# bioinfomaticsCSU/deepsignal

Measured on AMD Instinct MI355X. Metric: CpG sites/sec (batch=512, k=17, sig=360), higher is better.
Workload: dtype f32; 1 GPU; configs[1]: 1xMI355X, batch=512, random-init CpG model weights, synthetic (17,360) features, fp32; batch=512, kmer_len=17, signal_len=360

## Files before the change

deepsignal_amd/csrc/ds_kernels.hip:

```cpp
#include "ds_device.h"

namespace ds {


constexpr int DR_SLOTS = 4;
constexpr int DR_DIST = 3;
constexpr int DR_STAGE = 6 * 256;
constexpr int DR_A_FLOATS = 2 * 128 * (KC + 4);
constexpr int DR_LDS_FLOATS = DR_A_FLOATS + DR_SLOTS * DR_STAGE + 2 * 256;
constexpr int DR_SOLO_PAD_BYTES = 56 * 1024;

__device__ __forceinline__ void dr_gload4(v4f& dst, unsigned voff, const void* sbase)
{
    asm volatile("global_load_dwordx4 %0, %1, %2" : "=&v"(dst) : "v"(voff), "s"(sbase) : "memory");
}
template <int E> __device__ __forceinline__ float dr_elem(const v4f& v) { return E == 0 ? v.x : E == 1 ? v.y : E == 2 ? v.z : v.w; }

__device__ __forceinline__ void dense_ring_loop(const GemmProblem& P, float* smem, int m0, int tid, int lane, int wave,
                                                int t0, int t1, int t2, floatx16 (&acc)[1][3])
{
    constexpr int LDA = KC + 4;
    const int nchunks = P.K / KC;
    if (nchunks <= 0) return;
    float* const ring = smem + DR_A_FLOATS;
// ... 1788 lines not shown
    const int W = a.W, spt = a.spt;
    const int trows = spt * (W + 2) + 3;
    int* const rowmap = reinterpret_cast<int*>(T + trows * S23_LDT);
    const int site0 = blockIdx.x * spt;
    const int nhere = min(spt, a.n_sites - site0);
    const int TRv = nhere * W;
    const size_t grow0 = (size_t)site0 * W;
    const int h4 = 4 * (lane >> 5), rlane = lane & 31;

    for (int i = tid; i < trows * (S23_LDT / 4); i += 512) reinterpret_cast<float4*>(T)[i] = make_float4(0.f, 0.f, 0.f, 0.f);
    if (tid < 96) rowmap[tid] = tid < TRv ? (tid / W) * (W + 2) + 1 + tid % W : spt * (W + 2) + 1;
    {
        float4 v[3];
#pragma unroll
        for (int i = 0; i < 3; ++i) {
            const int idx = tid + 512 * i, row = idx >> 4, q = idx & 15;
            const int rr = row < TRv ? row : TRv - 1;
            v[i] = gload4(a.X + (grow0 + rr) * 64 + q * 4);
        }
#pragma unroll
        for (int i = 0; i < 3; ++i) {
            const int idx = tid + 512 * i, row = idx >> 4, q = idx & 15;
            *reinterpret_cast<float4*>(Xs + row * S23_LDX + q * 4) = v[i];
        }
    }
    const char* const b3 = reinterpret_cast<const char*>(a.Bp3) + (size_t)wave * 48 * 1024;
    const unsigned lane16 = (unsigned)lane * 16;
    float4 bq[4];
#pragma unroll
    for (int i = 0; i < 4; ++i) bq[i] = gload4(reinterpret_cast<const float*>(b3 + i * 1024 + lane16));
    float4 bias3[4];
#pragma unroll
    for (int g = 0; g < 4; ++g) bias3[g] = gload4(a.bias3 + wave * 32 + 8 * g + h4);
    __syncthreads();

    {
        const int n2 = wave & 3;
        float4 w2[8];
#pragma unroll
        for (int g = 0; g < 8; ++g) w2[g] = gload4(a.Bp2 + ((size_t)(n2 * 8 + g) * 64 + lane) * 4);
        float4 bias2[4];
#pragma unroll
        for (int g = 0; g < 4; ++g) bias2[g] = gload4(a.bias2 + n2 * 32 + 8 * g + h4);
        const int nunits = wave < 4 ? 2 : 1;
        for (int ui = 0; ui < nunits; ++ui) {
            const int m = wave < 4 ? 2 * ui : 1;
            floatx16 u;
#pragma unroll
            for (int g = 0; g < 4; ++g) { u[4 * g] = bias2[g].x; u[4 * g + 1] = bias2[g].y; u[4 * g + 2] = bias2[g].z; u[4 * g + 3] = bias2[g].w; }
            const float* xr = Xs + (m * 32 + rlane) * S23_LDX + h4;
#pragma unroll
            for (int g = 0; g < 8; ++g) {
                const float4 x = *reinterpret_cast<const float4*>(xr + g * 8);
                u = __builtin_amdgcn_mfma_f32_32x32x2f32(w2[g].x, x.x, u, 0, 0, 0);
                u = __builtin_amdgcn_mfma_f32_32x32x2f32(w2[g].y, x.y, u, 0, 0, 0);
                u = __builtin_amdgcn_mfma_f32_32x32x2f32(w2[g].z, x.z, u, 0, 0, 0);
                u = __builtin_amdgcn_mfma_f32_32x32x2f32(w2[g].w, x.w, u, 0, 0, 0);
            }
            const int row = m * 32 + rlane;
            float* const td = T + rowmap[row] * S23_LDT + n2 * 32 + h4;
#pragma unroll
            for (int g = 0; g < 4; ++g) {
                const float4 o = make_float4(relu_f(u[4 * g]), relu_f(u[4 * g + 1]), relu_f(u[4 * g + 2]), relu_f(u[4 * g + 3]));
                *reinterpret_cast<float4*>(td + 8 * g) = o;
                if (a.C2 && row < TRv) {
                    const v4f ov = {o.x, o.y, o.z, o.w};
                    *(__attribute__((address_space(1))) v4f*)(a.C2 + (grow0 + row) * 128 + n2 * 32 + 8 * g + h4) = ov;
                }
            }
        }
    }
    __syncthreads();

    floatx16 acc[3];
#pragma unroll
    for (int m = 0; m < 3; ++m)
#pragma unroll
        for (int g = 0; g < 4; ++g) { acc[m][4 * g] = bias3[g].x; acc[m][4 * g + 1] = bias3[g].y; acc[m][4 * g + 2] = bias3[g].z; acc[m][4 * g + 3] = bias3[g].w; }
    const float* tb[3];
#pragma unroll
    for (int m = 0; m < 3; ++m) tb[m] = T + (rowmap[m * 32 + rlane] - 1) * S23_LDT + h4;
    float4 af[2][3];
#pragma unroll
    for (int m = 0; m < 3; ++m) af[0][m] = *reinterpret_cast<const float4*>(tb[m]);
#pragma unroll
    for (int kgl = 0; kgl < 48; ++kgl) {
        const int cur = kgl & 1, slot = kgl & 3;
        if (kgl + 1 < 48) {
            const int t1 = (kgl + 1) >> 4, g1 = (kgl + 1) & 15;
#pragma unroll
            for (int m = 0; m < 3; ++m) af[cur ^ 1][m] = *reinterpret_cast<const float4*>(tb[m] + t1 * S23_LDT + g1 * 8);
        }
#pragma unroll
        for (int m = 0; m < 3; ++m) {
            acc[m] = __builtin_amdgcn_mfma_f32_32x32x2f32(bq[slot].x, af[cur][m].x, acc[m], 0, 0, 0);
            acc[m] = __builtin_amdgcn_mfma_f32_32x32x2f32(bq[slot].y, af[cur][m].y, acc[m], 0, 0, 0);
            acc[m] = __builtin_amdgcn_mfma_f32_32x32x2f32(bq[slot].z, af[cur][m].z, acc[m], 0, 0, 0);
            acc[m] = __builtin_amdgcn_mfma_f32_32x32x2f32(bq[slot].w, af[cur][m].w, acc[m], 0, 0, 0);
        }
        if (kgl + 4 < 48) bq[slot] = gload4(reinterpret_cast<const float*>(b3 + (kgl + 4) * 1024 + lane16));
        __builtin_amdgcn_sched_barrier(0);
    }

#pragma unroll
    for (int m = 0; m < 3; ++m) {
        const int row = m * 32 + rlane;
        if (row < TRv) {
            float* const yd = a.Y + (grow0 + row) * 256 + wave * 32 + h4;
#pragma unroll
            for (int g = 0; g < 4; ++g) {
                const v4f o = {relu_f(acc[m][4 * g]), relu_f(acc[m][4 * g + 1]), relu_f(acc[m][4 * g + 2]), relu_f(acc[m][4 * g + 3])};
                *(__attribute__((address_space(1))) v4f*)(yd + 8 * g) = o;
            }
        }
    }
}

hipError_t launch_stem23(const Stem23Args& a, hipStream_t s)
{
    if (a.n_sites <= 0) return hipSuccess;
    const int grid = (a.n_sites + a.spt - 1) / a.spt;
    hipLaunchKernelGGL(stem23_kernel, dim3(grid), dim3(512), stem23_lds_bytes(a.W, a.spt), s, a);
    return hipGetLastError();
}

constexpr int SB_LDX = 36;
constexpr int SB_LDT = 68;
constexpr int SB_LDO = 132;
size_t stem23_bf16_lds_bytes(int W, int spt)
{
    const size_t work = (size_t)96 * SB_LDX + (size_t)(spt * (W + 2) + 3) * SB_LDT;
    const size_t outt = (size_t)96 * SB_LDO;
    return ((work > outt ? work : outt) + 96) * sizeof(float);
}

__global__ __launch_bounds__(512, 4) void stem23_bf16_kernel(const Stem23Args a)
{
    extern __shared__ __attribute__((aligned(16))) float smem[];
    float* const Xs = smem;
    float* const T = smem + 96 * SB_LDX;
    float* const Ot = smem;
    const int tid = threadIdx.x, lane = tid & 63, wave = __builtin_amdgcn_readfirstlane(tid >> 6);
    const int W = a.W, spt = a.spt;
    const int trows = spt * (W + 2) + 3;
    const size_t work = (size_t)96 * SB_LDX + (size_t)trows * SB_LDT, outt = (size_t)96 * SB_LDO;
    int* const rowmap = reinterpret_cast<int*>(smem + (work > outt ? work : outt));
    const int site0 = blockIdx.x * spt;
    const int TRv = min(spt, a.n_sites - site0) * W;
    const size_t grow0 = (size_t)site0 * W;
    const int h4 = 4 * (lane >> 5), rlane = lane & 31;
    unsigned short* const Th = reinterpret_cast<unsigned short*>(T);
    unsigned short* const Oh = reinterpret_cast<unsigned short*>(Ot);
    auto pack4 = [](float x0, float x1, float x2, float x3) -> uint2 {
        return make_uint2(pack_bf2(relu_f(x0), relu_f(x1)), pack_bf2(relu_f(x2), relu_f(x3)));
    };

    for (int i = tid; i < trows * (SB_LDT / 4); i += 512) reinterpret_cast<float4*>(T)[i] = make_float4(0.f, 0.f, 0.f, 0.f);
    if (tid < 96) rowmap[tid] = tid < TRv ? (tid / W) * (W + 2) + 1 + tid % W : spt * (W + 2) + 1;
    {
        float4 v[2];
#pragma unroll
        for (int i = 0; i < 2; ++i) {
            const int idx = tid + 512 * i, row = idx >> 3, q = idx & 7;
            const int rr = row < TRv ? row : TRv - 1;
            if (idx < 768) v[i] = gload4(a.X + (grow0 + rr) * 32 + q * 4);
        }
#pragma unroll
        for (int i = 0; i < 2; ++i) {
            const int idx = tid + 512 * i, row = idx >> 3, q = idx & 7;
            if (idx < 768) *reinterpret_cast<float4*>(Xs + row * SB_LDX + q * 4) = v[i];
        }
    }
    const char* const b3 = reinterpret_cast<const char*>(a.Bp3) + (size_t)wave * 24 * 1024;
    const unsigned lane16 = (unsigned)lane * 16;
    float4 bq[4];
#pragma unroll
    for (int i = 0; i < 4; ++i) bq[i] = gload4(reinterpret_cast<const float*>(b3 + i * 1024 + lane16));
    float4 bias3[4];
#pragma unroll
    for (int g = 0; g < 4; ++g) bias3[g] = gload4(a.bias3 + wave * 32 + 8 * g + h4);
    __syncthreads();

    {
        const int n2 = wave & 3;
        float4 w2[4];
#pragma unroll
        for (int g = 0; g < 4; ++g) w2[g] = gload4(a.Bp2 + ((size_t)(n2 * 4 + g) * 64 + lane) * 4);
        float4 bias2[4];
#pragma unroll
        for (int g = 0; g < 4; ++g) bias2[g] = gload4(a.bias2 + n2 * 32 + 8 * g + h4);
        const int nunits = wave < 4 ? 2 : 1;
        for (int ui = 0; ui < nunits; ++ui) {
            const int m = wave < 4 ? 2 * ui : 1;
            floatx16 u;
#pragma unroll
            for (int g = 0; g < 4; ++g) { u[4 * g] = bias2[g].x; u[4 * g + 1] = bias2[g].y; u[4 * g + 2] = bias2[g].z; u[4 * g + 3] = bias2[g].w; }
            const float* xr = Xs + (m * 32 + rlane) * SB_LDX + h4;
#pragma unroll
            for (int g = 0; g < 4; ++g) u = mfma_bf(w2[g], *reinterpret_cast<const float4*>(xr + g * 8), u);
            const int row = m * 32 + rlane;
            unsigned short* const td = Th + rowmap[row] * (2 * SB_LDT) + n2 * 32 + h4;
#pragma unroll
            for (int g = 0; g < 4; ++g) {
                const uint2 o = pack4(u[4 * g], u[4 * g + 1], u[4 * g + 2], u[4 * g + 3]);
                *reinterpret_cast<uint2*>(td + 8 * g) = o;
                if (a.C2 && row < TRv) {
                    typedef unsigned int u2v __attribute__((ext_vector_type(2)));
                    const u2v ov = {o.x, o.y};
                    *(__attribute__((address_space(1))) u2v*)(reinterpret_cast<unsigned short*>(a.C2) + (grow0 + row) * 128 + n2 * 32 + 8 * g + h4) = ov;
                }
            }
        }
    }
    __syncthreads();

    floatx16 acc[3];
#pragma unroll
    for (int m = 0; m < 3; ++m)
#pragma unroll
        for (int g = 0; g < 4; ++g) { acc[m][4 * g] = bias3[g].x; acc[m][4 * g + 1] = bias3[g].y; acc[m][4 * g + 2] = bias3[g].z; acc[m][4 * g + 3] = bias3[g].w; }
    const float* tb[3];
#pragma unroll
    for (int m = 0; m < 3; ++m) tb[m] = T + (rowmap[m * 32 + rlane] - 1) * SB_LDT + h4;
    float4 af[3];
#pragma unroll
    for (int m = 0; m < 3; ++m) af[m] = *reinterpret_cast<const float4*>(tb[m]);
#pragma unroll
    for (int ks = 0; ks < 24; ++ks) {
        const int slot = ks & 3;
#pragma unroll
        for (int m = 0; m < 3; ++m) acc[m] = mfma_bf(bq[slot], af[m], acc[m]);
        if (ks + 4 < 24) bq[slot] = gload4(reinterpret_cast<const float*>(b3 + (ks + 4) * 1024 + lane16));
        if (ks + 1 < 24) {
            const int t1 = (ks + 1) >> 3, g1 = (ks + 1) & 7;
#pragma unroll
            for (int m = 0; m < 3; ++m) af[m] = *reinterpret_cast<const float4*>(tb[m] + t1 * SB_LDT + g1 * 8);
        }
        __builtin_amdgcn_sched_barrier(0);
    }
    __syncthreads();

#pragma unroll
    for (int m = 0; m < 3; ++m)
#pragma unroll
        for (int g = 0; g < 4; ++g)
            *reinterpret_cast<uint2*>(Oh + (m * 32 + rlane) * (2 * SB_LDO) + wave * 32 + 8 * g + h4) =
                pack4(acc[m][4 * g], acc[m][4 * g + 1], acc[m][4 * g + 2], acc[m][4 * g + 3]);
    __syncthreads();
    __attribute__((address_space(1))) unsigned short* const Yg =
        (__attribute__((address_space(1))) unsigned short*)(reinterpret_cast<unsigned short*>(a.Y) + grow0 * 256);
    for (int idx = tid; idx < 96 * 32; idx += 512) {
        const int row = idx >> 5, q = idx & 31;
        if (row < TRv) {
            const float4 v = *reinterpret_cast<const float4*>(Ot + row * SB_LDO + q * 4);
            v4f o = {v.x, v.y, v.z, v.w};
            *(__attribute__((address_space(1))) v4f*)(Yg + (unsigned)(row * 256 + q * 8)) = o;
        }
    }
}

hipError_t launch_stem23_bf16(const Stem23Args& a, hipStream_t s)
{
    if (a.n_sites <= 0) return hipSuccess;
    const int grid = (a.n_sites + a.spt - 1) / a.spt;
    hipLaunchKernelGGL(stem23_bf16_kernel, dim3(grid), dim3(512), stem23_bf16_lds_bytes(a.W, a.spt), s, a);
    return hipGetLastError();
}

hipError_t configure_fused_kernels()
{
    const void* fns[6] = {(const void*)inception_fused_kernel<1>, (const void*)inception_fused_kernel<2>,
                          (const void*)inception_fused_kernel<3>, (const void*)inception_fused_bf16_kernel<1>,
                          (const void*)inception_fused_bf16_kernel<2>, (const void*)inception_fused_bf16_kernel<3>};
    for (const void* f : fns) {
        const hipError_t e = hipFuncSetAttribute(f, hipFuncAttributeMaxDynamicSharedMemorySize, 160 * 1024);
        if (e != hipSuccess) return e;
    }
    const hipError_t e1 = hipFuncSetAttribute((const void*)gemm_kernel<1, 3, 4, 1, 0, 2, 2, 1>, hipFuncAttributeMaxDynamicSharedMemorySize, DR_SOLO_PAD_BYTES);
    if (e1 != hipSuccess) return e1;
    const hipError_t e2 = hipFuncSetAttribute((const void*)stem23_bf16_kernel, hipFuncAttributeMaxDynamicSharedMemorySize, (int)STEM23_MAX_LDS);
    if (e2 != hipSuccess) return e2;
    return hipFuncSetAttribute((const void*)stem23_kernel, hipFuncAttributeMaxDynamicSharedMemorySize, (int)STEM23_MAX_LDS);
}

hipError_t launch_inception_fused_bf16(int tm, const FusedChain& c, hipStream_t s)
{
    if (!fused_chain_ok(c)) return hipErrorInvalidValue;
    const FusedArgs& a = c.m[0];
    if (a.n_sites <= 0) return hipSuccess;
    for (int i = 1; i < c.nmod; ++i)
        if (c.m[i].cin != a.cin) return hipErrorInvalidValue;
    const size_t lds = inception_fused_bf16_lds_bytes(tm, a.W, a.spt);
    const int grid = (a.n_sites + a.spt - 1) / a.spt;
    switch (tm) {
    case 1: hipLaunchKernelGGL(inception_fused_bf16_kernel<1>, dim3(grid), dim3(512), lds, s, c); break;
    case 2: hipLaunchKernelGGL(inception_fused_bf16_kernel<2>, dim3(grid), dim3(512), lds, s, c); break;
    case 3: hipLaunchKernelGGL(inception_fused_bf16_kernel<3>, dim3(grid), dim3(512), lds, s, c); break;
    default: return hipErrorInvalidValue;
    }
    return hipGetLastError();
}

constexpr int STEM_HALO = 8;
template <bool OUT_BF>
__global__ __launch_bounds__(256) void stem1_kernel(const float* __restrict__ signals, const float* __restrict__ w,
                                                     const float* __restrict__ bias, float* __restrict__ out,
                                                     int signal_len, int w1, int pad_l_conv, int wa, int pad_l_pool)
{
    extern __shared__ __attribute__((aligned(16))) float sig[];
    const int site = blockIdx.x;
    const int total = signal_len + 2 * STEM_HALO + 8;
    for (int i = threadIdx.x; i < total; i += blockDim.x) {
        const int k = i - STEM_HALO;
        sig[i] = (k >= 0 && k < signal_len) ? signals[(size_t)site * signal_len + k] : 0.0f;
    }
    __syncthreads();
    const int c = threadIdx.x & 63;
    float wk[7];
#pragma unroll
    for (int t = 0; t < 7; ++t) wk[t] = w[t * 64 + c];
    const float b = bias[c];
    for (int p = threadIdx.x >> 6; p < wa; p += blockDim.x >> 6) {
        const int wc0 = 2 * p - pad_l_pool;
        const float* s0 = sig + STEM_HALO + 2 * wc0 - pad_l_conv;
        float v[11];
#pragma unroll
        for (int i = 0; i < 11; ++i) v[i] = s0[i];
        float best = -INFINITY;
#pragma unroll
        for (int pt = 0; pt < 3; ++pt) {
            float a = 0.0f;
#pragma unroll
            for (int t = 0; t < 7; ++t) a = fmaf(v[2 * pt + t], wk[t], a);
            const int wc = wc0 + pt;
            best = (wc >= 0 && wc < w1) ? __builtin_elementwise_maximum(best, a) : best;
        }
        const float y = relu_f(best + b);
        if (OUT_BF) reinterpret_cast<unsigned short*>(out)[((size_t)site * wa + p) * 64 + c] = f2bf(y);
        else out[((size_t)site * wa + p) * 64 + c] = y;
    }
}

hipError_t launch_stem1(const float* signals, const float* w7x64, const float* bias64, float* out, int n,
                        int signal_len, int w1, int pad_l_conv, int wa, int pad_l_pool, int out_bf16, hipStream_t s)
{
    if (n <= 0) return hipSuccess;
    const size_t lds = (signal_len + 2 * STEM_HALO + 8) * sizeof(float);
    if (lds > 64 * 1024) return hipErrorInvalidValue;
    if (out_bf16)
        hipLaunchKernelGGL(stem1_kernel<true>, dim3(n), dim3(256), lds, s, signals, w7x64, bias64, out,
                           signal_len, w1, pad_l_conv, wa, pad_l_pool);
    else
        hipLaunchKernelGGL(stem1_kernel<false>, dim3(n), dim3(256), lds, s, signals, w7x64, bias64, out,
                           signal_len, w1, pad_l_conv, wa, pad_l_pool);
    return hipGetLastError();
}

__global__ __launch_bounds__(256) void maxpool_s2_kernel(const float4* __restrict__ in, float4* __restrict__ out,
                                                          long total, int win, int wout, int pad_l, int ch4)
{
    for (long i = blockIdx.x * (long)blockDim.x + threadIdx.x; i < total; i += (long)gridDim.x * blockDim.x) {
        const int c = (int)(i % ch4);
        const long r = i / ch4;
        const int wo = (int)(r % wout);
        const long site = r / wout;
        float4 m = make_float4(0.0f, 0.0f, 0.0f, 0.0f);
#pragma unroll
        for (int t = 0; t < 3; ++t) {
            const int wi = 2 * wo + t - pad_l;
            if (wi >= 0 && wi < win) m = f4max_relu(m, in[(site * win + wi) * ch4 + c]);
        }
        out[i] = m;
    }
}

hipError_t launch_maxpool_s2(const float* in, float* out, int n, int win, int wout, int pad_l, int ch, hipStream_t s)
{
    const long total = (long)n * wout * (ch / 4);
    if (total <= 0) return hipSuccess;
    const int blocks = (int)((total + 255) / 256 < 4096 ? (total + 255) / 256 : 4096);
    hipLaunchKernelGGL(maxpool_s2_kernel, dim3(blocks), dim3(256), 0, s, (const float4*)in, (float4*)out, total, win, wout,
                       pad_l, ch / 4);
    return hipGetLastError();
}

__global__ __launch_bounds__(256) void avgpool7_kernel(const float4* __restrict__ in, float4* __restrict__ out, long total,
                                                        int w, int ch4)
{
    for (long i = blockIdx.x * (long)blockDim.x + threadIdx.x; i < total; i += (long)gridDim.x * blockDim.x) {
        const int c = (int)(i % ch4);
        const long r = i / ch4;
        const int wo = (int)(r % w);
        const long site = r / w;
        float4 a = make_float4(0.f, 0.f, 0.f, 0.f);
        int cnt = 0;
        for (int t = -3; t <= 3; ++t) {
            const int wi = wo + t;
            if (wi < 0 || wi >= w) continue;
            const float4 v = in[(site * w + wi) * ch4 + c];
            a.x += v.x; a.y += v.y; a.z += v.z; a.w += v.w;
            ++cnt;
        }
        const float d = (float)cnt;
        out[i] = make_float4(a.x / d, a.y / d, a.z / d, a.w / d);
    }
}

hipError_t launch_avgpool7(const float* in, float* out, int n, int w, int ch, hipStream_t s)
{
    const long total = (long)n * w * (ch / 4);
    if (total <= 0) return hipSuccess;
    const int blocks = (int)((total + 255) / 256 < 4096 ? (total + 255) / 256 : 4096);
    hipLaunchKernelGGL(avgpool7_kernel, dim3(blocks), dim3(256), 0, s, (const float4*)in, (float4*)out, total, w, ch / 4);
    return hipGetLastError();
}

__global__ __launch_bounds__(256) void head_kernel(const float* __restrict__ fc1, const float* __restrict__ w2,
                                                    float* __restrict__ logits, float* __restrict__ act,
                                                    int* __restrict__ pred, int n, int J, int C, int nparts, size_t part_stride)
{
    __shared__ float part[4][16];
    const int site = blockIdx.x;
    const int tid = threadIdx.x, lane = tid & 63, wave = tid >> 6;
    const float4* x4 = reinterpret_cast<const float4*>(fc1 + (size_t)site * J);
    float accv[16];
#pragma unroll
    for (int c = 0; c < 16; ++c) accv[c] = 0.0f;
    const int J4 = J >> 2;
    for (int k4 = tid; k4 < J4; k4 += 256) {
        float4 x = x4[k4];
        for (int p = 1; p < nparts; ++p) {
            const float4 y = *reinterpret_cast<const float4*>(fc1 + p * part_stride + (size_t)site * J + 4 * (size_t)k4);
            x.x += y.x; x.y += y.y; x.z += y.z; x.w += y.w;
        }
        const float* w = w2 + (size_t)k4 * 4 * C;
        if (C == 2) {
            const float4 wa = *reinterpret_cast<const float4*>(w);
            const float4 wb = *reinterpret_cast<const float4*>(w + 4);
            accv[0] = fmaf(x.x, wa.x, fmaf(x.y, wa.z, fmaf(x.z, wb.x, fmaf(x.w, wb.z, accv[0]))));
            accv[1] = fmaf(x.x, wa.y, fmaf(x.y, wa.w, fmaf(x.z, wb.y, fmaf(x.w, wb.w, accv[1]))));
        } else {
#pragma unroll
            for (int c = 0; c < 16; ++c)
                if (c < C) accv[c] += x.x * w[c] + x.y * w[C + c] + x.z * w[2 * C + c] + x.w * w[3 * C + c];
        }
    }
    for (int k = (J4 << 2) + tid; k < J; k += 256) {
        float xk = fc1[(size_t)site * J + k];
        for (int p = 1; p < nparts; ++p) xk += fc1[p * part_stride + (size_t)site * J + k];
        for (int c = 0; c < C; ++c) accv[c] += xk * w2[(size_t)k * C + c];
    }
#pragma unroll
    for (int c = 0; c < 16; ++c) {
        if (c >= C) break;
        float a = accv[c];
#pragma unroll
        for (int off = 32; off > 0; off >>= 1) a += __shfl_xor(a, off);
        if (lane == 0) part[wave][c] = a;
    }
    __syncthreads();
    if (tid == 0) {
        float best = 0.0f;
        int bi = 0;
        for (int c = 0; c < C; ++c) {
            const float a = (part[0][c] + part[1][c]) + (part[2][c] + part[3][c]);
            const float sg = sigmoidf_(a);
            logits[(size_t)site * C + c] = a;
            act[(size_t)site * C + c] = sg;
            if (c == 0 || sg > best) { best = sg; bi = c; }
        }
        pred[site] = bi;
    }
}

hipError_t launch_head(const float* fc1, const float* w2, float* logits, float* act, int* pred, int n, int J,
                       int class_num, hipStream_t s, int nparts, size_t part_stride)
{
    if (n <= 0) return hipSuccess;
    hipLaunchKernelGGL(head_kernel, dim3(n), dim3(256), 0, s, fc1, w2, logits, act, pred, n, J, class_num, nparts, part_stride);
    return hipGetLastError();
}

__global__ __launch_bounds__(256) void head_folded_kernel(const HeadFoldedArgs a)
{
    __shared__ float part[4][16];
    const int site = blockIdx.x, C = a.C;
    const int tid = threadIdx.x, lane = tid & 63, wave = tid >> 6;
    float accv[16];
#pragma unroll
    for (int c = 0; c < 16; ++c) accv[c] = 0.0f;
    int koff = 0;
    if (a.bf16) {
        for (int sg = 0; sg < a.nseg; ++sg) {
        const float4* x8 = reinterpret_cast<const float4*>(reinterpret_cast<const unsigned short*>(a.seg[sg]) + (size_t)site * a.pitch[sg]);
        for (int k8 = tid; k8 < (a.len[sg] >> 3); k8 += 256) {
            const float4 raw = x8[k8];
            const unsigned u[4] = {__float_as_uint(raw.x), __float_as_uint(raw.y), __float_as_uint(raw.z), __float_as_uint(raw.w)};
            const float* w = a.w + (size_t)(koff + k8 * 8) * C;
            if (C == 2) {
#pragma unroll
                for (int e = 0; e < 4; ++e) {
                    const float x0 = __uint_as_float(u[e] << 16), x1 = __uint_as_float(u[e] & 0xffff0000u);
                    const float4 wv = *reinterpret_cast<const float4*>(w + 4 * e);
                    accv[0] = fmaf(x0, wv.x, fmaf(x1, wv.z, accv[0]));
                    accv[1] = fmaf(x0, wv.y, fmaf(x1, wv.w, accv[1]));
                }
            } else {
#pragma unroll
                for (int e = 0; e < 4; ++e) {
                    const float x0 = __uint_as_float(u[e] << 16), x1 = __uint_as_float(u[e] & 0xffff0000u);
#pragma unroll
                    for (int c = 0; c < 16; ++c)
                        if (c < C) accv[c] += x0 * w[(2 * e) * C + c] + x1 * w[(2 * e + 1) * C + c];
                }
            }
        }
        koff += a.len[sg];
        }
    } else
    for (int sg = 0; sg < a.nseg; ++sg) {
        const int len = a.len[sg];
        const float4* x4 = reinterpret_cast<const float4*>(a.seg[sg] + (size_t)site * len);
        for (int k4 = tid; k4 < (len >> 2); k4 += 256) {
            const float4 x = x4[k4];
            const float* w = a.w + (size_t)(koff + k4 * 4) * C;
            if (C == 2) {
                const float4 wa = *reinterpret_cast<const float4*>(w);
                const float4 wb = *reinterpret_cast<const float4*>(w + 4);
                accv[0] = fmaf(x.x, wa.x, fmaf(x.y, wa.z, fmaf(x.z, wb.x, fmaf(x.w, wb.z, accv[0]))));
                accv[1] = fmaf(x.x, wa.y, fmaf(x.y, wa.w, fmaf(x.z, wb.y, fmaf(x.w, wb.w, accv[1]))));
            } else {
#pragma unroll
                for (int c = 0; c < 16; ++c)
                    if (c < C) accv[c] += x.x * w[c] + x.y * w[C + c] + x.z * w[2 * C + c] + x.w * w[3 * C + c];
            }
        }
        koff += len;
    }
#pragma unroll
    for (int c = 0; c < 16; ++c) {
        if (c >= C) break;
        float v = accv[c];
#pragma unroll
        for (int off = 32; off > 0; off >>= 1) v += __shfl_xor(v, off);
        if (lane == 0) part[wave][c] = v;
    }
    __syncthreads();
    if (tid == 0) {
        float best = 0.0f;
        int bi = 0;
        for (int c = 0; c < C; ++c) {
            const float v = (part[0][c] + part[1][c]) + (part[2][c] + part[3][c]);
            const float sgm = sigmoidf_(v);
            a.logits[(size_t)site * C + c] = v;
            a.act[(size_t)site * C + c] = sgm;
            if (c == 0 || sgm > best) { best = sgm; bi = c; }
        }
        a.pred[site] = bi;
    }
}

hipError_t launch_head_folded(const HeadFoldedArgs& a, hipStream_t s)
{
    if (a.n <= 0) return hipSuccess;
    hipLaunchKernelGGL(head_folded_kernel, dim3(a.n), dim3(256), 0, s, a);
    return hipGetLastError();
}

__global__ __launch_bounds__(256) void gather_inputs_kernel(const int* __restrict__ kmer, const float* __restrict__ means,
                                                            const float* __restrict__ stds, const float* __restrict__ lens,
                                                            const float* __restrict__ signals, float* __restrict__ block,
                                                            int n, int T, int S, int B, long lo, long hi)
{
    const long nt = (long)n * T;
    const long bt = (long)B * T;
    for (long i = lo + (long)blockIdx.x * 256 + threadIdx.x; i < hi; i += (long)gridDim.x * 256) {
        if (i < nt) reinterpret_cast<int*>(block)[i] = kmer[i];
        else if (i < 2 * nt) block[bt + (i - nt)] = means[i - nt];
        else if (i < 3 * nt) block[2 * bt + (i - 2 * nt)] = stds[i - 2 * nt];
        else if (i < 4 * nt) block[3 * bt + (i - 3 * nt)] = lens[i - 3 * nt];
        else block[4 * bt + (i - 4 * nt)] = signals[i - 4 * nt];
    }
}

__global__ __launch_bounds__(256) void scatter_outputs_kernel(const float* __restrict__ act, const int* __restrict__ pred,
                                                              float* __restrict__ act_out, int* __restrict__ pred_out, int n, int C)
{
    const int total = n * C + n;
    for (int i = blockIdx.x * 256 + threadIdx.x; i < total; i += gridDim.x * 256) {
        if (i < n * C) act_out[i] = act[i];
        else pred_out[i - n * C] = pred[i - n * C];
    }
}

hipError_t launch_gather_inputs(const int* kmer, const float* means, const float* stds, const float* lens, const float* signals,
                                float* block, int n, int T, int S, int B, int col_lo, int col_hi, hipStream_t s)
{
    if (n <= 0 || col_lo < 0 || col_hi > 4 * T + S || col_lo >= col_hi) return hipSuccess;
    const long lo = (long)n * col_lo, hi = (long)n * col_hi;
    const int grid = (int)std::min<long>((hi - lo + 1023) / 1024, 1024);
    hipLaunchKernelGGL(gather_inputs_kernel, dim3(grid), dim3(256), 0, s, kmer, means, stds, lens, signals, block, n, T, S, B, lo, hi);
    return hipGetLastError();
}

hipError_t launch_scatter_outputs(const float* act, const int* pred, float* act_out, int* pred_out, int n, int C, hipStream_t s)
{
    if (n <= 0) return hipSuccess;
    hipLaunchKernelGGL(scatter_outputs_kernel, dim3((n * (C + 1) + 255) / 256), dim3(256), 0, s, act, pred, act_out, pred_out, n, C);
    return hipGetLastError();
}

__global__ __launch_bounds__(256) void maxpool_s2_bf16_kernel(const float4* __restrict__ in, float4* __restrict__ out,
                                                               long total, int win, int wout, int pad_l, int ch8)
{
    for (long i = blockIdx.x * (long)blockDim.x + threadIdx.x; i < total; i += (long)gridDim.x * blockDim.x) {
        const int c = (int)(i % ch8);
        const long r = i / ch8;
        const int wo = (int)(r % wout);
        const long site = r / wout;
        float4 m = make_float4(0.0f, 0.0f, 0.0f, 0.0f);
#pragma unroll
        for (int t = 0; t < 3; ++t) {
            const int wi = 2 * wo + t - pad_l;
            if (wi >= 0 && wi < win) m = bf8max_relu(m, in[(site * win + wi) * ch8 + c]);
        }
        out[i] = m;
    }
}

hipError_t launch_maxpool_s2_bf16(const float* in, float* out, int n, int win, int wout, int pad_l, int ch_ld, hipStream_t s)
{
    const long total = (long)n * wout * (ch_ld / 8);
    if (total <= 0) return hipSuccess;
    const int blocks = (int)((total + 255) / 256 < 8192 ? (total + 255) / 256 : 8192);
    hipLaunchKernelGGL(maxpool_s2_bf16_kernel, dim3(blocks), dim3(256), 0, s, (const float4*)in, (float4*)out, total, win,
                       wout, pad_l, ch_ld / 8);
    return hipGetLastError();
}

__global__ __launch_bounds__(256) void avgpool7_bf16_kernel(const float4* __restrict__ in, unsigned short* __restrict__ out,
                                                             long total, int w, int ch8, int ld_in8, long out_ld, int out_off)
{
    for (long i = blockIdx.x * (long)blockDim.x + threadIdx.x; i < total; i += (long)gridDim.x * blockDim.x) {
        const int c = (int)(i % ch8);
        const long r = i / ch8;
        const int wo = (int)(r % w);
        const long site = r / w;
        float a[8] = {0, 0, 0, 0, 0, 0, 0, 0};
        int cnt = 0;
        for (int t = -3; t <= 3; ++t) {
            const int wi = wo + t;
            if (wi < 0 || wi >= w) continue;
            const float4 v = in[(site * w + wi) * ld_in8 + c];
            const unsigned u[4] = {__float_as_uint(v.x), __float_as_uint(v.y), __float_as_uint(v.z), __float_as_uint(v.w)};
#pragma unroll
            for (int q = 0; q < 4; ++q) {
                a[2 * q] += __uint_as_float(u[q] << 16);
                a[2 * q + 1] += __uint_as_float(u[q] & 0xffff0000u);
            }
            ++cnt;
        }
        const float d = (float)cnt;
        unsigned o[4];
#pragma unroll
        for (int q = 0; q < 4; ++q) o[q] = pack_bf2(a[2 * q] / d, a[2 * q + 1] / d);
        *reinterpret_cast<uint4*>(out + site * out_ld + out_off + ((long)wo * ch8 + c) * 8) = make_uint4(o[0], o[1], o[2], o[3]);
    }
}

hipError_t launch_avgpool7_bf16(const float* in, float* joint, int n, int w, int ch, int ld_in, int joint_ld, int joint_off,
                                hipStream_t s)
{
    const long total = (long)n * w * (ch / 8);
    if (total <= 0) return hipSuccess;
    const int blocks = (int)((total + 255) / 256 < 8192 ? (total + 255) / 256 : 8192);
    hipLaunchKernelGGL(avgpool7_bf16_kernel, dim3(blocks), dim3(256), 0, s, (const float4*)in, (unsigned short*)joint, total, w,
                       ch / 8, ld_in / 8, (long)joint_ld, joint_off);
    return hipGetLastError();
}

template <bool SRC_BF>
__global__ __launch_bounds__(256) void pack_event_feat_bf16_kernel(const float* __restrict__ hfw, const float* __restrict__ hbw,
                                                                    unsigned short* __restrict__ joint, int n, long joint_ld)
{
    const long i = blockIdx.x * (long)blockDim.x + threadIdx.x;
    if (i >= (long)n * 128) return;
    const int site = (int)(i / 128), q = (int)(i % 128);
    uint2 o;
    if (SRC_BF) {
        const unsigned short* src = reinterpret_cast<const unsigned short*>(q < 64 ? hfw : hbw) + (size_t)site * 256 + (q & 63) * 4;
        o = *reinterpret_cast<const uint2*>(src);
    } else {
        const float* src = (q < 64 ? hfw : hbw) + (size_t)site * 256 + (q & 63) * 4;
        const float4 v = *reinterpret_cast<const float4*>(src);
        o = make_uint2(pack_bf2(v.x, v.y), pack_bf2(v.z, v.w));
    }
    *reinterpret_cast<uint2*>(joint + site * joint_ld + q * 4) = o;
}

hipError_t launch_pack_event_feat_bf16(const float* hfw, const float* hbw, float* joint, int n, int joint_ld, int src_bf16,
                                       hipStream_t s)
{
    if (n <= 0) return hipSuccess;
    const dim3 grid((unsigned)(((long)n * 128 + 255) / 256));
    if (src_bf16)
        hipLaunchKernelGGL(pack_event_feat_bf16_kernel<true>, grid, dim3(256), 0, s, hfw, hbw, (unsigned short*)joint, n, (long)joint_ld);
    else
        hipLaunchKernelGGL(pack_event_feat_bf16_kernel<false>, grid, dim3(256), 0, s, hfw, hbw, (unsigned short*)joint, n, (long)joint_ld);
    return hipGetLastError();
}

__global__ __launch_bounds__(256) void embed_table_kernel(const float* __restrict__ emb, const float* __restrict__ kernel,
                                                           float* __restrict__ table, int vocab, int esize, int ncol)
{
    const long i = blockIdx.x * (long)blockDim.x + threadIdx.x;
    if (i >= (long)vocab * ncol) return;
    const int col = (int)(i % ncol);
    const int v = (int)(i / ncol);
    float a = 0.0f;
    for (int e = 0; e < esize; ++e) a = fmaf(emb[(size_t)v * esize + e], kernel[(size_t)e * ncol + col], a);
    table[i] = a;
}

hipError_t launch_embed_table(const float* emb, const float* kernel, float* table, int vocab, int esize, int ncol,
                              hipStream_t s)
{
    const long total = (long)vocab * ncol;
    hipLaunchKernelGGL(embed_table_kernel, dim3((unsigned)((total + 255) / 256)), dim3(256), 0, s, emb, kernel, table, vocab,
                       esize, ncol);
    return hipGetLastError();
}

}
```

Measured before the change: 461,300 sites/s.

## Restructure small kernels: stem1 carry reuse, per-site avgpool, segment-wise gather copies, wave priority

Rewrites several small auxiliary kernels. stem1 now gives each wave a contiguous range of pool outputs and reuses the overlapping conv result and sliding signal window. avgpool7 runs one block per site without per-element div/mod. Gather and scatter become per-segment vectorized uint4 copies. Several kernels raise wave priority with s_setprio and use 32-bit byte offsets for addressing. The aim is to cut index arithmetic and instruction overhead in these minor stages, at the cost of added complexity and new overflow and alignment assumptions.

Measured after the change: 466,800 sites/s, median of 6. +1.2%, better.

```diff
diff --git a/deepsignal_amd/csrc/ds_kernels.hip b/deepsignal_amd/csrc/ds_kernels.hip
--- a/deepsignal_amd/csrc/ds_kernels.hip
+++ b/deepsignal_amd/csrc/ds_kernels.hip
@@ -2114,17 +2114,29 @@
 }
 
 constexpr int STEM_HALO = 8;
+#ifndef DS_SMALL_PRIO
+#define DS_SMALL_PRIO 1
+#endif
+#ifndef DS_SMALL_PRIO_POST
+#define DS_SMALL_PRIO_POST 0
+#endif
+template <typename T> __device__ __forceinline__ T* at_bytes(T* base, unsigned bytes)
+{
+    return (T*)((const char*)base + bytes);
+}
+constexpr int STEM1_WAVES = 4;
 template <bool OUT_BF>
 __global__ __launch_bounds__(256) void stem1_kernel(const float* __restrict__ signals, const float* __restrict__ w,
                                                      const float* __restrict__ bias, float* __restrict__ out,
                                                      int signal_len, int w1, int pad_l_conv, int wa, int pad_l_pool)
 {
     extern __shared__ __attribute__((aligned(16))) float sig[];
-    const int site = blockIdx.x;
+    if constexpr (!OUT_BF && DS_SMALL_PRIO != 0) __builtin_amdgcn_s_setprio(DS_SMALL_PRIO);
     const int total = signal_len + 2 * STEM_HALO + 8;
+    const float* src = signals + (size_t)blockIdx.x * signal_len;
     for (int i = threadIdx.x; i < total; i += blockDim.x) {
         const int k = i - STEM_HALO;
-        sig[i] = (k >= 0 && k < signal_len) ? signals[(size_t)site * signal_len + k] : 0.0f;
+        sig[i] = (k >= 0 && k < signal_len) ? *at_bytes(src, 4u * (unsigned)k) : 0.0f;
     }
     __syncthreads();
     const int c = threadIdx.x & 63;
@@ -2132,25 +2144,44 @@
 #pragma unroll
     for (int t = 0; t < 7; ++t) wk[t] = w[t * 64 + c];
     const float b = bias[c];
-    for (int p = threadIdx.x >> 6; p < wa; p += blockDim.x >> 6) {
-        const int wc0 = 2 * p - pad_l_pool;
-        const float* s0 = sig + STEM_HALO + 2 * wc0 - pad_l_conv;
+    const int wave = __builtin_amdgcn_readfirstlane(threadIdx.x >> 6);
+    const int chunk = (wa + STEM1_WAVES - 1) / STEM1_WAVES;
+    const int p_lo = wave * chunk, p_hi = p_lo + chunk < wa ? p_lo + chunk : wa;
+    if (p_lo < p_hi) {
+        const float* s0 = sig + STEM_HALO + 2 * (2 * p_lo - pad_l_pool) - pad_l_conv;
+        float* orow = out + (size_t)blockIdx.x * wa * (OUT_BF ? 32 : 64);
         float v[11];
 #pragma unroll
-        for (int i = 0; i < 11; ++i) v[i] = s0[i];
-        float best = -INFINITY;
-#pragma unroll
-        for (int pt = 0; pt < 3; ++pt) {
-            float a = 0.0f;
-#pragma unroll
-            for (int t = 0; t < 7; ++t) a = fmaf(v[2 * pt + t], wk[t], a);
-            const int wc = wc0 + pt;
-            best = (wc >= 0 && wc < w1) ? __builtin_elementwise_maximum(best, a) : best;
-        }
-        const float y = relu_f(best + b);
-        if (OUT_BF) reinterpret_cast<unsigned short*>(out)[((size_t)site * wa + p) * 64 + c] = f2bf(y);
-        else out[((size_t)site * wa + p) * 64 + c] = y;
-    }
+        for (int i = 0; i < 7; ++i) v[i] = s0[i];
+        float carry = 0.0f;
+#pragma unroll
+        for (int t = 0; t < 7; ++t) carry = fmaf(v[t], wk[t], carry);
+        for (int p = p_lo; p < p_hi; ++p, s0 += 4) {
+#pragma unroll
+            for (int i = 7; i < 11; ++i) v[i] = s0[i];
+            const int wc0 = 2 * p - pad_l_pool;
+            float best = -INFINITY;
+#pragma unroll
+            for (int pt = 0; pt < 3; ++pt) {
+                float a = carry;
+                if (pt > 0) {
+                    a = 0.0f;
+#pragma unroll
+                    for (int t = 0; t < 7; ++t) a = fmaf(v[2 * pt + t], wk[t], a);
+                }
+                const int wc = wc0 + pt;
+                best = (wc >= 0 && wc < w1) ? __builtin_elementwise_maximum(best, a) : best;
+                if (pt == 2) carry = a;
+            }
+            const float y = relu_f(best + b);
+            const unsigned o = (unsigned)p * 64u + (unsigned)c;
+            if (OUT_BF) *at_bytes(reinterpret_cast<unsigned short*>(orow), 2u * o) = f2bf(y);
+            else *at_bytes(orow, 4u * o) = y;
+#pragma unroll
+            for (int i = 0; i < 7; ++i) v[i] = v[i + 4];
+        }
+    }
+    if constexpr (!OUT_BF && DS_SMALL_PRIO != 0) __builtin_amdgcn_s_setprio(0);
 }
 
 hipError_t launch_stem1(const float* signals, const float* w7x64, const float* bias64, float* out, int n,
@@ -2160,10 +2191,10 @@
     const size_t lds = (signal_len + 2 * STEM_HALO + 8) * sizeof(float);
     if (lds > 64 * 1024) return hipErrorInvalidValue;
     if (out_bf16)
-        hipLaunchKernelGGL(stem1_kernel<true>, dim3(n), dim3(256), lds, s, signals, w7x64, bias64, out,
+        hipLaunchKernelGGL(stem1_kernel<true>, dim3(n), dim3(64 * STEM1_WAVES), lds, s, signals, w7x64, bias64, out,
                            signal_len, w1, pad_l_conv, wa, pad_l_pool);
     else
-        hipLaunchKernelGGL(stem1_kernel<false>, dim3(n), dim3(256), lds, s, signals, w7x64, bias64, out,
+        hipLaunchKernelGGL(stem1_kernel<false>, dim3(n), dim3(64 * STEM1_WAVES), lds, s, signals, w7x64, bias64, out,
                            signal_len, w1, pad_l_conv, wa, pad_l_pool);
     return hipGetLastError();
 }
@@ -2196,34 +2227,33 @@
     return hipGetLastError();
 }
 
-__global__ __launch_bounds__(256) void avgpool7_kernel(const float4* __restrict__ in, float4* __restrict__ out, long total,
-                                                        int w, int ch4)
-{
-    for (long i = blockIdx.x * (long)blockDim.x + threadIdx.x; i < total; i += (long)gridDim.x * blockDim.x) {
-        const int c = (int)(i % ch4);
-        const long r = i / ch4;
-        const int wo = (int)(r % w);
-        const long site = r / w;
-        float4 a = make_float4(0.f, 0.f, 0.f, 0.f);
-        int cnt = 0;
-        for (int t = -3; t <= 3; ++t) {
-            const int wi = wo + t;
-            if (wi < 0 || wi >= w) continue;
-            const float4 v = in[(site * w + wi) * ch4 + c];
-            a.x += v.x; a.y += v.y; a.z += v.z; a.w += v.w;
-            ++cnt;
-        }
-        const float d = (float)cnt;
-        out[i] = make_float4(a.x / d, a.y / d, a.z / d, a.w / d);
-    }
+__global__ __launch_bounds__(256) void avgpool7_kernel(const float4* __restrict__ in, float4* __restrict__ out, int w, int ch4)
+{
+    if constexpr (DS_SMALL_PRIO != 0) __builtin_amdgcn_s_setprio(DS_SMALL_PRIO);
+    const size_t base = (size_t)blockIdx.x * (size_t)w * (size_t)ch4;
+    const float4* src = in + base;
+    float4* dst = out + base;
+    const int lane = threadIdx.x & 63, wave = __builtin_amdgcn_readfirstlane(threadIdx.x >> 6);
+    for (int wo = wave; wo < w; wo += 4) {
+        const int lo = wo - 3 > 0 ? wo - 3 : 0, hi = wo + 3 < w - 1 ? wo + 3 : w - 1;
+        const float d = (float)(hi - lo + 1);
+        for (int c = lane; c < ch4; c += 64) {
+            float4 a = make_float4(0.f, 0.f, 0.f, 0.f);
+            for (int wi = lo; wi <= hi; ++wi) {
+                const float4 v = *at_bytes(src, 16u * (unsigned)(wi * ch4 + c));
+                a.x += v.x; a.y += v.y; a.z += v.z; a.w += v.w;
+            }
+            *at_bytes(dst, 16u * (unsigned)(wo * ch4 + c)) = make_float4(a.x / d, a.y / d, a.z / d, a.w / d);
+        }
+    }
+    if constexpr (DS_SMALL_PRIO != 0) __builtin_amdgcn_s_setprio(0);
 }
 
 hipError_t launch_avgpool7(const float* in, float* out, int n, int w, int ch, hipStream_t s)
 {
-    const long total = (long)n * w * (ch / 4);
-    if (total <= 0) return hipSuccess;
-    const int blocks = (int)((total + 255) / 256 < 4096 ? (total + 255) / 256 : 4096);
-    hipLaunchKernelGGL(avgpool7_kernel, dim3(blocks), dim3(256), 0, s, (const float4*)in, (float4*)out, total, w, ch / 4);
+    if (n <= 0 || w <= 0 || ch < 4) return hipSuccess;
+    if ((long)w * (ch / 4) >= (1L << 27)) return hipErrorInvalidValue;
+    hipLaunchKernelGGL(avgpool7_kernel, dim3(n), dim3(256), 0, s, (const float4*)in, (float4*)out, w, ch / 4);
     return hipGetLastError();
 }
 
@@ -2232,20 +2262,24 @@
                                                     int* __restrict__ pred, int n, int J, int C, int nparts, size_t part_stride)
 {
     __shared__ float part[4][16];
+    if constexpr (DS_SMALL_PRIO_POST != 0) __builtin_amdgcn_s_setprio(DS_SMALL_PRIO_POST);
     const int site = blockIdx.x;
     const int tid = threadIdx.x, lane = tid & 63, wave = tid >> 6;
-    const float4* x4 = reinterpret_cast<const float4*>(fc1 + (size_t)site * J);
+    const char* xrow = reinterpret_cast<const char*>(fc1 + (size_t)site * J);
+    const char* wrow = reinterpret_cast<const char*>(w2);
+    const size_t part_bytes = part_stride * sizeof(float);
     float accv[16];
 #pragma unroll
     for (int c = 0; c < 16; ++c) accv[c] = 0.0f;
     const int J4 = J >> 2;
     for (int k4 = tid; k4 < J4; k4 += 256) {
-        float4 x = x4[k4];
+        const unsigned xo = (unsigned)k4 * 16u;
+        float4 x = *reinterpret_cast<const float4*>(at_bytes(xrow, xo));
         for (int p = 1; p < nparts; ++p) {
-            const float4 y = *reinterpret_cast<const float4*>(fc1 + p * part_stride + (size_t)site * J + 4 * (size_t)k4);
+            const float4 y = *reinterpret_cast<const float4*>(at_bytes(xrow + p * part_bytes, xo));
             x.x += y.x; x.y += y.y; x.z += y.z; x.w += y.w;
         }
-        const float* w = w2 + (size_t)k4 * 4 * C;
+        const float* w = reinterpret_cast<const float*>(wrow + xo * (unsigned)C);
         if (C == 2) {
             const float4 wa = *reinterpret_cast<const float4*>(w);
             const float4 wb = *reinterpret_cast<const float4*>(w + 4);
@@ -2258,9 +2292,10 @@
         }
     }
     for (int k = (J4 << 2) + tid; k < J; k += 256) {
-        float xk = fc1[(size_t)site * J + k];
-        for (int p = 1; p < nparts; ++p) xk += fc1[p * part_stride + (size_t)site * J + k];
-        for (int c = 0; c < C; ++c) accv[c] += xk * w2[(size_t)k * C + c];
+        const unsigned ko = (unsigned)k * 4u;
+        float xk = *reinterpret_cast<const float*>(xrow + ko);
+        for (int p = 1; p < nparts; ++p) xk += *reinterpret_cast<const float*>(xrow + p * part_bytes + ko);
+        for (int c = 0; c < C; ++c) accv[c] += xk * *reinterpret_cast<const float*>(wrow + (ko * (unsigned)C + 4u * (unsigned)c));
     }
 #pragma unroll
     for (int c = 0; c < 16; ++c) {
@@ -2283,6 +2318,7 @@
         }
         pred[site] = bi;
     }
+    if constexpr (DS_SMALL_PRIO_POST != 0) __builtin_amdgcn_s_setprio(0);
 }
 
 hipError_t launch_head(const float* fc1, const float* w2, float* logits, float* act, int* pred, int n, int J,
@@ -2296,6 +2332,7 @@
 __global__ __launch_bounds__(256) void head_folded_kernel(const HeadFoldedArgs a)
 {
     __shared__ float part[4][16];
+    if constexpr (DS_SMALL_PRIO_POST != 0) __builtin_amdgcn_s_setprio(DS_SMALL_PRIO_POST);
     const int site = blockIdx.x, C = a.C;
     const int tid = threadIdx.x, lane = tid & 63, wave = tid >> 6;
     float accv[16];
@@ -2304,11 +2341,12 @@
     int koff = 0;
     if (a.bf16) {
         for (int sg = 0; sg < a.nseg; ++sg) {
-        const float4* x8 = reinterpret_cast<const float4*>(reinterpret_cast<const unsigned short*>(a.seg[sg]) + (size_t)site * a.pitch[sg]);
+        const char* x8 = reinterpret_cast<const char*>(reinterpret_cast<const unsigned short*>(a.seg[sg]) + (size_t)site * a.pitch[sg]);
+        const char* wseg = reinterpret_cast<const char*>(a.w + (size_t)koff * C);
         for (int k8 = tid; k8 < (a.len[sg] >> 3); k8 += 256) {
-            const float4 raw = x8[k8];
+            const float4 raw = *reinterpret_cast<const float4*>(x8 + (unsigned)k8 * 16u);
             const unsigned u[4] = {__float_as_uint(raw.x), __float_as_uint(raw.y), __float_as_uint(raw.z), __float_as_uint(raw.w)};
-            const float* w = a.w + (size_t)(koff + k8 * 8) * C;
+            const float* w = reinterpret_cast<const float*>(wseg + (unsigned)k8 * 32u * (unsigned)C);
             if (C == 2) {
 #pragma unroll
                 for (int e = 0; e < 4; ++e) {
@@ -2332,10 +2370,12 @@
     } else
     for (int sg = 0; sg < a.nseg; ++sg) {
         const int len = a.len[sg];
-        const float4* x4 = reinterpret_cast<const float4*>(a.seg[sg] + (size_t)site * len);
+        const char* x4 = reinterpret_cast<const char*>(a.seg[sg] + (size_t)site * len);
+        const char* wseg = reinterpret_cast<const char*>(a.w + (size_t)koff * C);
         for (int k4 = tid; k4 < (len >> 2); k4 += 256) {
-            const float4 x = x4[k4];
-            const float* w = a.w + (size_t)(koff + k4 * 4) * C;
+            const unsigned xo = (unsigned)k4 * 16u;
+            const float4 x = *reinterpret_cast<const float4*>(x4 + xo);
+            const float* w = reinterpret_cast<const float*>(wseg + xo * (unsigned)C);
             if (C == 2) {
                 const float4 wa = *reinterpret_cast<const float4*>(w);
                 const float4 wb = *reinterpret_cast<const float4*>(w + 4);
@@ -2370,6 +2410,7 @@
         }
         a.pred[site] = bi;
     }
+    if constexpr (DS_SMALL_PRIO_POST != 0) __builtin_amdgcn_s_setprio(0);
 }
 
 hipError_t launch_head_folded(const HeadFoldedArgs& a, hipStream_t s)
@@ -2379,30 +2420,50 @@
     return hipGetLastError();
 }
 
+__device__ __forceinline__ void copy_words(const unsigned* __restrict__ src, unsigned* __restrict__ dst, long cnt)
+{
+    const unsigned tid = threadIdx.x;
+    const long step = (long)gridDim.x * 256;
+    if (((reinterpret_cast<uintptr_t>(src) | reinterpret_cast<uintptr_t>(dst)) & 15) == 0) {
+        const long cnt4 = cnt >> 2;
+        for (long i0 = (long)blockIdx.x * 256; i0 < cnt4; i0 += step) {
+            const unsigned left = (unsigned)(cnt4 - i0 < 256 ? cnt4 - i0 : 256);
+            if (tid < left) (reinterpret_cast<uint4*>(dst) + i0)[tid] = (reinterpret_cast<const uint4*>(src) + i0)[tid];
+        }
+        if (blockIdx.x == 0 && tid < (unsigned)(cnt & 3)) (dst + 4 * cnt4)[tid] = (src + 4 * cnt4)[tid];
+    } else {
+        for (long i0 = (long)blockIdx.x * 256; i0 < cnt; i0 += step) {
+            const unsigned left = (unsigned)(cnt - i0 < 256 ? cnt - i0 : 256);
+            if (tid < left) (dst + i0)[tid] = (src + i0)[tid];
+        }
+    }
+}
+
 __global__ __launch_bounds__(256) void gather_inputs_kernel(const int* __restrict__ kmer, const float* __restrict__ means,
                                                             const float* __restrict__ stds, const float* __restrict__ lens,
                                                             const float* __restrict__ signals, float* __restrict__ block,
-                                                            int n, int T, int S, int B, long lo, long hi)
-{
+                                                            int n, int T, int S, int B, long lo, long hi, int seg0)
+{
+    if constexpr (DS_SMALL_PRIO != 0) __builtin_amdgcn_s_setprio(DS_SMALL_PRIO);
     const long nt = (long)n * T;
     const long bt = (long)B * T;
-    for (long i = lo + (long)blockIdx.x * 256 + threadIdx.x; i < hi; i += (long)gridDim.x * 256) {
-        if (i < nt) reinterpret_cast<int*>(block)[i] = kmer[i];
-        else if (i < 2 * nt) block[bt + (i - nt)] = means[i - nt];
-        else if (i < 3 * nt) block[2 * bt + (i - 2 * nt)] = stds[i - 2 * nt];
-        else if (i < 4 * nt) block[3 * bt + (i - 3 * nt)] = lens[i - 3 * nt];
-        else block[4 * bt + (i - 4 * nt)] = signals[i - 4 * nt];
-    }
+    const int seg = seg0 + (int)blockIdx.y;
+    const void* arr = seg == 0 ? (const void*)kmer : seg == 1 ? (const void*)means : seg == 2 ? (const void*)stds
+                    : seg == 3 ? (const void*)lens : (const void*)signals;
+    const long first = seg * nt, last = seg < 4 ? first + nt : first + (long)n * S;
+    const long from = lo > first ? lo : first, to = hi < last ? hi : last;
+    if (from < to)
+        copy_words(static_cast<const unsigned*>(arr) + (from - first), reinterpret_cast<unsigned*>(block) + seg * bt + (from - first), to - from);
+    if constexpr (DS_SMALL_PRIO != 0) __builtin_amdgcn_s_setprio(0);
 }
 
 __global__ __launch_bounds__(256) void scatter_outputs_kernel(const float* __restrict__ act, const int* __restrict__ pred,
                                                               float* __restrict__ act_out, int* __restrict__ pred_out, int n, int C)
 {
-    const int total = n * C + n;
-    for (int i = blockIdx.x * 256 + threadIdx.x; i < total; i += gridDim.x * 256) {
-        if (i < n * C) act_out[i] = act[i];
-        else pred_out[i - n * C] = pred[i - n * C];
-    }
+    if constexpr (DS_SMALL_PRIO_POST != 0) __builtin_amdgcn_s_setprio(DS_SMALL_PRIO_POST);
+    if (blockIdx.y == 0) copy_words(reinterpret_cast<const unsigned*>(act), reinterpret_cast<unsigned*>(act_out), (long)n * C);
+    else copy_words(reinterpret_cast<const unsigned*>(pred), reinterpret_cast<unsigned*>(pred_out), n);
+    if constexpr (DS_SMALL_PRIO_POST != 0) __builtin_amdgcn_s_setprio(0);
 }
 
 hipError_t launch_gather_inputs(const int* kmer, const float* means, const float* stds, const float* lens, const float* signals,
@@ -2410,15 +2471,19 @@
 {
     if (n <= 0 || col_lo < 0 || col_hi > 4 * T + S || col_lo >= col_hi) return hipSuccess;
     const long lo = (long)n * col_lo, hi = (long)n * col_hi;
-    const int grid = (int)std::min<long>((hi - lo + 1023) / 1024, 1024);
-    hipLaunchKernelGGL(gather_inputs_kernel, dim3(grid), dim3(256), 0, s, kmer, means, stds, lens, signals, block, n, T, S, B, lo, hi);
+    const int seg0 = std::min(col_lo / T, 4), seg1 = std::min((col_hi - 1) / T, 4);
+    const long widest = (long)n * (seg1 == 4 ? std::max(S, seg0 < 4 ? T : 0) : T);
+    const int grid = (int)std::min<long>((widest + 1023) / 1024, 1024);
+    hipLaunchKernelGGL(gather_inputs_kernel, dim3(grid, seg1 - seg0 + 1), dim3(256), 0, s, kmer, means, stds, lens, signals, block, n, T, S,
+                       B, lo, hi, seg0);
     return hipGetLastError();
 }
 
 hipError_t launch_scatter_outputs(const float* act, const int* pred, float* act_out, int* pred_out, int n, int C, hipStream_t s)
 {
     if (n <= 0) return hipSuccess;
-    hipLaunchKernelGGL(scatter_outputs_kernel, dim3((n * (C + 1) + 255) / 256), dim3(256), 0, s, act, pred, act_out, pred_out, n, C);
+    hipLaunchKernelGGL(scatter_outputs_kernel, dim3((int)std::min<long>(((long)n * C + 1023) / 1024, 1024), 2), dim3(256), 0, s, act, pred,
+                       act_out, pred_out, n, C);
     return hipGetLastError();
 }
 
```
